# happykygo/GNN-eCommerce

Hardware: AMD Instinct MI355X
Metric: edges propagated/sec per LGConv layer (higher is better)
Workload: dtype f32; 1 GPU; configs[1]: 1639358 users x 54571 items, 20314816 directed edges, 3 LGConv layers, emb_dim 64, get_embedding (K hops + fused layer sum); parallelism=single, seed=0

## Files before the change

### gnn-ecommerce_amd/_native.py

```python
from __future__ import annotations

import ctypes
import os
from ctypes import CFUNCTYPE, POINTER, Structure, c_char_p, c_float, c_int, c_int32, c_int64, c_size_t, c_uint64, c_void_p
from typing import Optional

import torch

LIB_NAME = "liblgconv_hip.so"
LIB_PATH = os.environ.get("LGCN_LIB_PATH") or os.path.join(os.path.dirname(os.path.abspath(__file__)), "csrc", LIB_NAME)
ABI_VERSION = 14

ST_INDEX_OOB = 1
ST_SAMPLER_EXHAUSTED = 2

class SweepCfg(Structure):
    _fields_ = [("n_bands", c_int32), ("waves_per_band_round", c_int32), ("row_cap", c_int32), ("piece_cap", c_int32),
                ("lookahead", c_int32), ("groups", c_int32), ("round_order", c_int32), ("light_len", c_int32)]


class SweepDims(Structure):
    _fields_ = [("n_bands", c_int32), ("rounds", c_int32), ("row_cap", c_int32), ("piece_cap", c_int32),
                ("n_rows", c_int32), ("groups", c_int32),
                ("n_waves", c_int64), ("n_slabs", c_int64), ("n_slots", c_int64), ("n_entries", c_int64),
# ... 57 lines not shown
                                    c_int64, c_void_p]),
    "lgc_bipartite_split": (c_int, [c_void_p, c_int64, c_void_p, c_void_p]),
    "lgc_row_plan_workspace_bytes": (c_size_t, [c_int64]),
    "lgc_row_plan_count": (c_int, [c_void_p, c_int32, c_int32, c_int32, c_int32, c_void_p, c_size_t, c_void_p, c_void_p]),
    "lgc_row_plan_fill": (c_int, [c_void_p, c_int32, c_int32, c_int32, c_int32, c_void_p, c_void_p, c_void_p, c_void_p]),
    "lgc_tile_classes_workspace_bytes": (c_size_t, [c_int64, c_int64]),
    "lgc_tile_classes": (c_int, [c_void_p, c_void_p, c_int32, c_int32, c_int32, c_int32, c_int64, c_void_p, c_size_t, c_void_p,
                                 c_void_p, c_void_p]),
    "lgc_tile_pack": (c_int, [c_void_p, c_void_p, c_int64, c_int32, c_void_p, c_void_p, c_void_p]),
    "lgc_build_tiles": (c_int, [c_void_p, c_void_p, c_void_p, c_int64, c_int32, c_void_p, c_void_p]),
    "lgc_spmm_tiles": (c_int, [c_void_p, c_void_p, c_void_p, c_int32, c_int32, c_int32, c_int64, c_void_p, c_int64,
                               c_void_p, c_int64, c_void_p, c_int64, c_float, c_float, c_int32, c_void_p]),
    "lgc_sweep_plan_create": (c_void_p, [c_void_p, c_void_p, c_int32, c_int32, c_int32, c_int32, POINTER(SweepCfg),
                                         POINTER(c_int)]),
    "lgc_sweep_plan_dims": (c_int, [c_void_p, POINTER(SweepDims)]),
    "lgc_sweep_plan_export": (c_int, [c_void_p, c_void_p, c_void_p, c_void_p, c_void_p, c_void_p]),
    "lgc_sweep_plan_upload": (c_int, [c_void_p, c_void_p, c_void_p, c_void_p, c_void_p, c_void_p]),
    "lgc_sweep_plan_export_multi": (c_int, [c_void_p, c_void_p]),
    "lgc_sweep_plan_free": (None, [c_void_p]),
    "lgc_sweep_dplan_workspace_bytes": (c_size_t, [c_int64, c_int64, c_int64, POINTER(SweepCfg)]),
    "lgc_sweep_dplan_create": (c_void_p, [c_void_p, c_void_p, c_int32, c_int32, c_int64, c_int64, c_int32, c_int32,
                                          POINTER(SweepCfg), c_void_p, c_size_t, c_void_p, POINTER(c_int)]),
    "lgc_sweep_dplan_dims": (c_int, [c_void_p, POINTER(SweepDims)]),
    "lgc_sweep_dplan_fill": (c_int, [c_void_p, c_void_p, c_void_p, c_void_p, c_void_p, c_void_p]),
    "lgc_sweep_dplan_export_multi": (c_int, [c_void_p, c_void_p]),
    "lgc_sweep_dplan_free": (None, [c_void_p]),
    "lgc_sweep_ok": (c_int, [c_int32, c_int64, c_int64]),
    "lgc_spmm_sweep": (c_int, [c_void_p, c_void_p, c_void_p, c_void_p, c_int64, c_int32, c_int32, c_void_p, c_int32, c_void_p,
                               c_int32, c_void_p, c_int64, c_void_p, c_int64, c_void_p, c_int64, c_void_p, c_int64, c_float, c_float,
                               c_int32, c_void_p]),
    "lgc_apply_route": (c_int, [POINTER(OperatorC), c_int64, c_int64, c_int64, c_int64, c_int32]),
    "lgc_apply": (c_int, [POINTER(OperatorC), c_int64, c_void_p, c_int64, c_void_p, c_int64, c_void_p, c_int64, c_float, c_float,
                          c_int32, c_void_p]),
    "lgc_hop_exchange": (c_int, [POINTER(OperatorC), POINTER(OperatorC), c_int64, c_void_p, c_int64, c_void_p, c_int64, c_void_p,
                                 c_int64, c_float, c_float, c_int32, c_int32, c_int32, c_int32, EXCHANGE_FN, c_void_p, c_void_p]),
    "lgc_segment_sum": (c_int, [c_void_p, c_void_p, c_void_p, c_void_p, c_int64, c_float, c_void_p, c_int64, c_int64, c_int32,
                                c_int32, c_void_p]),
    "lgc_pair_dot_rows": (c_int, [c_void_p, c_int64, c_int32, c_int64, c_void_p, c_void_p, c_int64, c_void_p, c_void_p, c_void_p,
                                  c_void_p, c_void_p, c_void_p]),
    "lgc_reg_rows": (c_int, [c_void_p, c_int64, c_int32, c_int64, c_void_p, c_int64, c_void_p, c_int64, c_void_p, c_int64, c_float,
                             c_void_p, c_void_p, c_void_p, c_void_p]),
    "lgc_bpr_loss": (c_int, [c_void_p, c_void_p, c_int64, c_int64, c_void_p, c_void_p, c_void_p]),
    "lgc_pair_seed_vals": (c_int, [c_void_p, c_void_p, c_void_p, c_void_p, c_void_p, c_int64, c_int32, c_void_p, c_void_p]),
    "lgc_seed_prepare": (c_int, [c_void_p, c_int64, c_int64, c_int64, c_void_p, c_void_p, c_void_p, c_void_p, c_void_p, c_void_p,
                                 c_void_p, c_void_p, c_void_p]),
    "lgc_seed_flags": (c_int, [c_void_p, c_int64, c_int64, c_void_p, c_int32, c_void_p]),
    "lgc_seed_pull": (c_int, [c_void_p, c_void_p, c_int32, c_int32, c_int32, c_void_p, c_int32, c_void_p, c_int32, c_void_p,
                              c_void_p, c_void_p, c_void_p, c_void_p, c_int64, c_int64, c_void_p, c_int64, c_int32, c_void_p]),
    "lgc_seed_mark": (c_int, [c_void_p, c_void_p, c_int32, c_int32, c_void_p, c_int64, c_void_p, c_int64, c_int32, c_void_p]),
    "lgc_adam_step": (c_int, [c_void_p, c_void_p, c_void_p, c_void_p, c_int64, c_float, c_float, c_float, c_float, c_float,
                              c_float, c_void_p]),
    "lgc_adam_step_hp": (c_int, [c_void_p, c_void_p, c_void_p, c_void_p, c_int64, c_void_p, c_void_p]),
    "lgc_lincomb": (c_int, [c_void_p, c_int64, c_void_p, c_void_p, c_void_p, c_int32, c_int64, c_int32, c_void_p]),
    "lgc_mask_topk": (c_int, [c_void_p, c_int64, c_void_p, c_int64, c_void_p, c_void_p, c_void_p, c_int64, c_int32, c_int32,
                              c_void_p, c_void_p, c_void_p]),
    "lgc_fold_in": (c_int, [c_void_p, c_void_p, c_void_p, c_int64, c_void_p, c_void_p, c_int64, c_int64, c_void_p, c_void_p,
                            c_int64, c_int64, c_float, c_int32, c_int32, c_void_p, c_int64, c_void_p, c_void_p]),
    "lgc_score_rows": (c_int, [c_void_p, c_int64, c_int64, c_void_p, c_int64, c_void_p, c_int64, c_int32, c_int32, c_void_p,
                               c_int64, c_void_p, c_void_p]),
    "lgc_topk_hits": (c_int, [c_void_p, c_int64, c_int32, c_void_p, c_void_p, c_void_p, c_int64, c_int64, c_void_p, c_void_p,
                              c_void_p, c_void_p]),
    "lgc_metric_sums": (c_int, [c_void_p, c_void_p, c_int64, c_void_p, c_void_p, c_void_p]),
    "lgc_rank_metrics": (c_int, [c_void_p, c_int64, c_int32, c_void_p, c_void_p, c_void_p, c_void_p, c_int64, c_int64,
                                 POINTER(c_int32), c_int32, c_void_p, c_void_p, c_void_p, c_void_p, c_void_p]),
    "lgc_column_sums": (c_int, [c_void_p, c_int64, c_int64, c_int32, c_void_p, c_void_p]),
    "lgc_topk_coverage": (c_int, [c_void_p, c_int64, c_int32, c_int64, POINTER(c_int32), c_int32, c_int64, c_void_p, c_void_p,
# ... 130 lines not shown
```

### gnn-ecommerce_amd/csrc/lgconv_hip.hip

```cpp
#include <hipcub/hipcub.hpp>

#include <cstdlib>
#include <cstdio>
#include <cstring>
#include <chrono>
#include <new>
#include <thread>
#include <type_traits>
#include <utility>
#include <vector>

#include "lgconv_common.h"

namespace {

__global__ void k_build_keys(const int64_t *__restrict__ edge_index, int64_t n_edges, int64_t n_nodes,
                             int by_source, int32_t *__restrict__ keys, int32_t *__restrict__ ids,
                             int32_t *__restrict__ status) {
    int64_t e = (int64_t)blockIdx.x * blockDim.x + threadIdx.x;
    if (e >= n_edges) return;
    int64_t src = edge_index[e], dst = edge_index[n_edges + e];
    bool ok = src >= 0 && src < n_nodes && dst >= 0 && dst < n_nodes;
    if (!ok) atomicOr(status, LGC_ST_INDEX_OOB);
    keys[e] = ok ? (int32_t)(by_source ? src : dst) : 0;
// ... 1192 lines not shown
        __syncthreads();
        if (wv == 0 && active && g == 0) {
            for (int o = 1; o < kBlock / kWave; ++o) {
#pragma unroll
                for (int i = 0; i < VEC; ++i) acc.v[i] = __fadd_rn(acc.v[i], wave_sum[o * 256 + l * VEC + i]);
            }
            Acc<VEC> rv;
            rv.zero();
            if (p.r != nullptr) rv = load_row<VEC>(p.r + (int64_t)mr.row * p.r_stride + c0);
            finish_row<VEC, SpmmArgs>(p, mr.row, c0, acc, rv);
        }
        return;
    }
    const int64_t m = (((int64_t)blockIdx.x - n_wide) * (kBlock / kWave) + wv) * groups + g;
    if (g >= groups || m >= n_multi) return;
    const lgc_multi_row mr = multi[m];
    Acc<VEC> acc, rv;
    acc.zero();
    rv.zero();
    if (p.r != nullptr) rv = load_row<VEC>(p.r + (int64_t)mr.row * p.r_stride + c0);
    for (int32_t s = mr.slot_begin; s < mr.slot_end; s += 8) {
        Acc<VEC> t[8];
#pragma unroll
        for (int j = 0; j < 8; ++j) {
            t[j].zero();
            if (s + j < mr.slot_end) t[j] = load_row<VEC>(pb + (int64_t)(s + j) * p.dim);
        }
#pragma unroll
        for (int j = 0; j < 8; ++j)
#pragma unroll
            for (int i = 0; i < VEC; ++i) acc.v[i] = __fadd_rn(acc.v[i], t[j].v[i]);
    }
    finish_row<VEC, SpmmArgs>(p, mr.row, c0, acc, rv);
}

__global__ void k_seed_mark(const int32_t *__restrict__ rowptr, const lgc_entry *__restrict__ entries, int32_t row_begin,
                            int32_t row_end, const int64_t *__restrict__ seed_rows, int64_t n_seed, uint8_t *__restrict__ mark,
                            int64_t mark_len, uint8_t value) {
    const int lane = threadIdx.x & (kWave - 1);
    const int64_t t = (int64_t)blockIdx.x * (blockDim.x / kWave) + threadIdx.x / kWave;
    if (t >= n_seed) return;
    const int64_t row = seed_rows[t];
    if (row < row_begin || row >= row_end) return;
    if (t > 0 && seed_rows[t - 1] == row) return;
    for (int32_t k = rowptr[row] + lane; k < rowptr[row + 1]; k += kWave) {
        const int32_t c = entries[k].col;
        if (c >= 0 && c < mark_len) mark[c] = value;
    }
}

__global__ void k_split_init(long long *__restrict__ out) {
    out[0] = -1;
    out[1] = 0x7FFFFFFFFFFFFFFFll;
}

__global__ __launch_bounds__(kBlock) void k_bipartite_split(const int64_t *__restrict__ edge_index, int64_t n_edges,
                                                           long long *__restrict__ out) {
    long long lo = -1, hi = 0x7FFFFFFFFFFFFFFFll;
    for (int64_t e = (int64_t)blockIdx.x * blockDim.x + threadIdx.x; e < n_edges; e += (int64_t)gridDim.x * blockDim.x) {
        const long long a = edge_index[e], b = edge_index[n_edges + e];
        lo = max(lo, min(a, b));
        hi = min(hi, max(a, b));
    }
#pragma unroll
    for (int off = kWave / 2; off > 0; off >>= 1) {
        lo = max(lo, (long long)__shfl_xor(lo, off));
// ... 1388 lines not shown
    };
    int rc = up(wave_slab_ptr, plan->wave_slab_ptr.data(), plan->wave_slab_ptr.size() * 4);
    if (rc == 0) rc = up(wave_npieces, plan->wave_npieces.data(), plan->wave_npieces.size() * 4);
    if (rc == 0) rc = up(piece_slot, plan->piece_slot.data(), plan->piece_slot.size() * 4);
    if (rc != 0) return rc;
    const lgc_sweep_cfg &cfg = plan->cfg;
    const int64_t n_waves = plan->dims.n_waves;
    if (n_waves > 0 && plan->dims.n_entries > 0) {
        const uint32_t pad_x = 0x00FFFFFFu | ((uint32_t)cfg.row_cap << 24);
        hipLaunchKernelGGL((k_dp_steps<true>), dim3(ceil_div(n_waves, kBlock / kWave)), dim3(kBlock), 0, st, plan->keys, plan->idx,
                           plan->sorted, plan->d_item_ptr, (int32_t)n_waves, plan->dims.groups, cfg.lookahead,
                           cfg.waves_per_band_round, cfg.n_bands, cfg.round_order == 2 ? 1 : 0, pad_x, (int32_t *)nullptr,
                           (int32_t *)nullptr, (const int32_t *)wave_slab_ptr, slabs);
    }
    rc = (int)hipGetLastError();
    if (rc != 0) return rc;
    return (int)hipStreamSynchronize(st);
}

void lgc_sweep_dplan_free(lgc_sweep_dplan *plan) { delete plan; }

static bool sweep_table_ok(int32_t dim, int64_t table_rows, int64_t x_stride) {
    if (table_rows <= 0 || table_rows >= 0xFFFFFF || x_stride < dim) return false;
    const int64_t bytes = table_bytes(table_rows, x_stride, dim);
    const uint32_t pad = (uint32_t)(0xFFFFFFull * (uint64_t)(x_stride * 4));
    return x_stride * 4 < (1 << 24) && bytes < (int64_t(1) << 32) && (int64_t)pad >= bytes;
}

int lgc_sweep_ok(int32_t dim, int64_t table_rows, int64_t x_stride) {
    const int groups = (dim >= 61 && dim <= 64) ? 4 : (dim >= 68 && dim <= kWideRow) ? 2 : (dim > kWideRow && dim <= 128) ? 4 : 0;
    return groups != 0 && sweep_table_ok(dim, table_rows, x_stride) ? groups : 0;
}

int lgc_spmm_sweep(const uint32_t *slabs, const int32_t *wave_slab_ptr, const int32_t *wave_npieces, const int32_t *piece_slot,
                   int64_t n_waves, int32_t row_cap, int32_t groups, const lgc_multi_row *multi, int32_t n_rows,
                   const lgc_multi_row *multi_wide, int32_t n_wide, float *partials,
                   int64_t table_rows, const float *x, int64_t x_stride, float *y, int64_t y_stride, const float *r,
                   int64_t r_stride, float a, float b, int32_t dim, void *stream_) {
    if (!slabs || !wave_slab_ptr || !wave_npieces || !piece_slot || !partials || !x || !y || n_waves < 0 ||
        n_waves % 4 != 0 || n_rows < 0 || n_wide < 0 || (n_rows > 0 && !multi) || (n_wide > 0 && !multi_wide) || row_cap < 1 ||
        row_cap > 254 || x == y)
        return LGC_E_INVAL;
    if (groups == 0) groups = 4;
    if (lgc_sweep_ok(dim, table_rows, x_stride) != groups) return LGC_E_DIM;
    if (const int rc = check_tables(x, x_stride, y, y_stride, r, r_stride, dim)) return rc;
    if (!aligned_to(slabs, 16) || !aligned_to(partials, 16)) return LGC_E_ALIGN;
    hipStream_t stream = as_stream(stream_);
    const size_t lds = (size_t)(kBlock / kWave) * (size_t)(row_cap + 1) * (groups == 2 ? kWideRow : 64) * sizeof(float);
    if (lds > 160 * 1024) return LGC_E_INVAL;
    if (n_waves > 0) {
        SweepArgs p{reinterpret_cast<const u4 *>(slabs), wave_slab_ptr, wave_npieces, piece_slot, x, partials, x_stride,
                    (uint32_t)table_bytes(table_rows, x_stride, dim), dim, row_cap, (int32_t)n_waves, 0, nullptr, dim, 0};
        const bool two_pass = groups == 4 && dim > 64;
        if (two_pass) {
            p.dim = 64;
            p.x_bytes = (uint32_t)table_bytes(table_rows, x_stride, 64);
        }
#ifdef LGC_SWEEP_TRACE
        if (const char *tr = getenv("LGCN_SWEEP_TRACE")) p.trace = reinterpret_cast<unsigned long long *>(strtoull(tr, nullptr, 0));
#endif
        static unsigned long long lds_ok_sweep = 0, lds_ok_wide = 0;
        int rc_attr = allow_big_lds(reinterpret_cast<const void *>(k_sweep<kSweepDepth>), 160 * 1024, &lds_ok_sweep);
        if (rc_attr == 0) rc_attr = allow_big_lds(reinterpret_cast<const void *>(k_sweep_wide<8>), 160 * 1024, &lds_ok_wide);
        if (rc_attr != 0) return rc_attr;
        const int64_t req = knobs().sweep_launch_waves;
        const int64_t per_launch = req > 0 ? std::max<int64_t>(4, (req / 4) * 4) : n_waves;
        for (int64_t w0 = 0; w0 < n_waves; w0 += per_launch) {
            p.wave_begin = (int32_t)w0;
            const unsigned blocks = (unsigned)(std::min<int64_t>(per_launch, n_waves - w0) / 4);
            if (groups == 2) hipLaunchKernelGGL(k_sweep_wide<8>, dim3(blocks), dim3(kBlock), lds, stream, p);
            else hipLaunchKernelGGL(k_sweep<kSweepDepth>, dim3(blocks), dim3(kBlock), lds, stream, p);
            if (two_pass) {
                SweepArgs q = p;
                q.x = x + 64;
                q.dim = dim - 64;
                q.x_bytes = (uint32_t)table_bytes(table_rows, x_stride, dim - 64);
                q.pcol = 64;
                hipLaunchKernelGGL(k_sweep<kSweepDepth>, dim3(blocks), dim3(kBlock), lds, stream, q);
            }
        }
    }
    DimCfg cfg;
    dim_cfg(dim, &cfg);
    SpmmArgs sp{nullptr, nullptr, x, y, r, x_stride, y_stride, r_stride, a, b, dim, cfg.lpr, 0, 0, 0, 0};
    sp.wt_store = wt_store_ok(table_rows, y_stride) ? 1 : 0;
    if (n_wide + n_rows > 0) {
        const int rows_per_block = (kBlock / kWave) * (kWave / cfg.lpr);
        hipLaunchKernelGGL((k_sweep_combine<4>), dim3(n_wide + ceil_div(n_rows, rows_per_block)), dim3(kBlock), 0, stream, sp,
                           multi_wide, n_wide, multi, n_rows, partials);
    }
    return (int)hipGetLastError();
}

int lgc_apply_route(const lgc_operator *op, int64_t table_rows, int64_t x_stride, int64_t y_stride, int64_t r_stride,
                    int32_t dim) {
    if (!op || op->n_tile_classes < 0 || op->n_tile_classes > 3) return LGC_E_INVAL;
    DimCfg cfg;
    if (!dim_cfg(dim, &cfg)) return LGC_E_DIM;
    if (table_rows < 0 || x_stride < dim || y_stride < dim || r_stride < 0 || (r_stride > 0 && r_stride < dim)) return LGC_E_INVAL;
    const int wt = wt_store_ok(table_rows, y_stride) ? LGC_ROUTE_WT_STORE : 0;
    if (op->sweep) {
        const int groups = op->sweep->groups ? op->sweep->groups : 4;
        if (lgc_sweep_ok(dim, table_rows, x_stride) == groups)
            return wt | (groups == 2 ? LGC_ROUTE_SWEEP_WIDE : dim > 64 ? LGC_ROUTE_SWEEP_TWO_PASS : LGC_ROUTE_SWEEP);
    }
    if (op->n_tile_classes == 0 || dim < 4) return wt | LGC_ROUTE_ROWS;
    bool fast = true;
    for (int c = 0; c < op->n_tile_classes; ++c)
        if (op->tiles[c].n_tiles != 0)
            fast = fast && tiles_fast_ok(op->tiles[c].meta != nullptr, dim, table_rows, x_stride, y_stride, r_stride);
    if (knobs().no_fused_apply) return wt | (fast ? LGC_ROUTE_SPLIT_DPP : LGC_ROUTE_SPLIT_GENERIC);
    return wt | (fast ? LGC_ROUTE_FUSED_DPP : LGC_ROUTE_FUSED_GENERIC);
}

int lgc_apply(const lgc_operator *op, int64_t table_rows, const float *x, int64_t x_stride, float *y, int64_t y_stride,
              const float *r, int64_t r_stride, float a, float b, int32_t dim, void *stream) {
    const int route = lgc_apply_route(op, table_rows, x_stride, y_stride, r ? r_stride : 0, dim);
    if (route < 0) return route;
    if (r && r_stride < dim) return LGC_E_INVAL;
    switch (route & ~LGC_ROUTE_WT_STORE) {
    case LGC_ROUTE_SWEEP:
    case LGC_ROUTE_SWEEP_WIDE:
    case LGC_ROUTE_SWEEP_TWO_PASS: {
        const lgc_sweep_arrays *sw = op->sweep;
// ... 35 lines not shown
        hipStream_t st = as_stream(stream);
        if (total > 0) {
            if (fast && dim > 64) hipLaunchKernelGGL((k_apply_fused<2>), dim3((unsigned)total), dim3(kBlock), 0, st, f);
            else if (fast) hipLaunchKernelGGL((k_apply_fused<1>), dim3((unsigned)total), dim3(kBlock), 0, st, f);
            else hipLaunchKernelGGL((k_apply_fused<0>), dim3((unsigned)total), dim3(kBlock), 0, st, f);
        }
        if (op->n_multi > 0)
            hipLaunchKernelGGL((k_spmm_combine<4>), dim3(ceil_div(op->n_multi, kBlock / kWave)), dim3(kBlock), 0, st, f.sp, op->multi,
                               op->n_multi, op->partials);
        return (int)hipGetLastError();
    }
    default:
        break;
    }
    const bool tiled = (route & ~LGC_ROUTE_WT_STORE) != LGC_ROUTE_ROWS;
    if (!tiled || op->n_chunks > 0) {
        const int rc = lgc_spmm(op->rowptr, op->entries, op->row_begin, tiled ? op->row_begin : op->row_end, op->short_max,
                                op->chunks, op->n_chunks, op->multi, op->n_multi, op->partials, table_rows, x, x_stride, y,
                                y_stride, r, r_stride, a, b, dim, stream);
        if (rc != 0) return rc;
    }
    if (tiled) {
        for (int c = 0; c < op->n_tile_classes; ++c) {
            const lgc_tile_class &tc = op->tiles[c];
            const int rc = lgc_spmm_tiles(tc.order, tc.meta, tc.slab, tc.n_tiles, tc.width,
                                          op->tiles_per_wave > 0 ? op->tiles_per_wave : 1, table_rows, x, x_stride, y,
                                          y_stride, r, r_stride, a, b, dim, stream);
            if (rc != 0) return rc;
        }
    }
    return 0;
}

int lgc_hop_exchange(const lgc_operator *item_op, const lgc_operator *user_op, int64_t table_rows, const float *x,
                     int64_t x_stride, float *y, int64_t y_stride, const float *r, int64_t r_stride, float a, float b,
                     int32_t dim, int32_t exchange_row_begin, int32_t exchange_rows, int32_t item_epilogue,
                     lgc_exchange_fn exchange, void *user, void *stream) {
    if (!item_op || !user_op || !exchange || exchange_row_begin < 0 || exchange_rows < 0 ||
        (int64_t)exchange_row_begin + exchange_rows > table_rows)
        return LGC_E_INVAL;
    int rc = lgc_apply(item_op, table_rows, x, x_stride, y, y_stride, item_epilogue ? r : nullptr, item_epilogue ? r_stride : 0, a,
                       item_epilogue ? b : 0.0f, dim, stream);
    if (rc != 0) return rc;
    rc = exchange(y + (int64_t)exchange_row_begin * y_stride, exchange_rows, y_stride, dim, stream, user);
    if (rc != 0) return rc;
    return lgc_apply(user_op, table_rows, x, x_stride, y, y_stride, r, r_stride, a, b, dim, stream);
}

int lgc_seed_mark(const int32_t *rowptr, const lgc_entry *entries, int32_t row_begin, int32_t row_end, const int64_t *seed_rows,
                  int64_t n_seed, uint8_t *mark, int64_t mark_len, int32_t value, void *stream_) {
    if (n_seed < 0 || row_begin < 0 || row_end < row_begin || mark_len < 0 || value < 0 || value > 255) return LGC_E_INVAL;
    if (n_seed == 0) return 0;
    if (!rowptr || !entries || !seed_rows || !mark) return LGC_E_INVAL;
    hipLaunchKernelGGL(k_seed_mark, dim3(ceil_div(n_seed, (int64_t)(kBlock / kWave))), dim3(kBlock), 0, as_stream(stream_), rowptr, entries,
                       row_begin, row_end, seed_rows, n_seed, mark, mark_len, (uint8_t)value);
    return (int)hipGetLastError();
}

int lgc_seed_pull(const int32_t *rowptr, const lgc_entry *entries, int32_t row_begin, int32_t row_end, int32_t short_max,
                  const lgc_chunk *chunks, int32_t n_chunks, const lgc_multi_row *multi, int32_t n_multi, float *partials,
                  const uint8_t *col_flag, const int32_t *col_slot, const uint8_t *row_mark, const float *seed_vals,
                  int64_t seed_stride, int64_t table_rows, float *y, int64_t y_stride, int32_t dim, void *stream_) {
    DimCfg cfg;
    if (!dim_cfg(dim, &cfg)) return LGC_E_DIM;
    if (!rowptr || !col_flag || !col_slot || row_begin < 0 || row_end < row_begin || n_chunks < 0 || n_multi < 0 ||
        short_max < 0 || table_rows < row_end)
// ... 50 lines not shown
```

### gnn-ecommerce_amd/graph.py

```python
from __future__ import annotations

import os
from collections import OrderedDict
from dataclasses import dataclass, field
from typing import Callable, Dict, List, Optional, Tuple

import torch
from torch import Tensor

from . import _native

SHORT_MAX = int(os.environ.get("LGCN_SHORT_MAX", "32"))
CHUNK_LEN = int(os.environ.get("LGCN_CHUNK_LEN", "256"))
USER_CHUNK_LEN = int(os.environ.get("LGCN_USER_CHUNK_LEN", "4096"))
TILE_WIDTHS = (8, 16, 32)
USE_TILES = os.environ.get("LGCN_TILES", "1") == "1"
TILES_PER_WAVE = int(os.environ.get("LGCN_TILES_PER_WAVE", "1"))
TILE_ORDER = os.environ.get("LGCN_TILE_ORDER", "cold")
USE_SWEEP = os.environ.get("LGCN_SWEEP", "auto")
SWEEP_MIN_ENTRIES = int(os.environ.get("LGCN_SWEEP_MIN_ENTRIES", "1000000"))
SWEEP_ADAPTIVE_BANDS = os.environ.get("LGCN_SWEEP_ADAPTIVE_BANDS", "1") == "1"
SWEEP_PIECE_ENTRIES = int(os.environ.get("LGCN_SWEEP_PIECE_ENTRIES", "20"))
SWEEP_CFG = dict(n_bands=int(os.environ.get("LGCN_SWEEP_BANDS", "8")), waves_per_band_round=int(os.environ.get("LGCN_SWEEP_WAVES", "256")),
                 row_cap=int(os.environ.get("LGCN_SWEEP_ROW_CAP", "78")),
# ... 488 lines not shown
                                      _native.ptr(sw.piece_slot), _native.ptr(sw.multi) if sw.multi.size(0) else None,
                                      _native.ptr(sw.multi_wide) if sw.multi_wide.size(0) else None,
                                      _native.ptr(sw.partials(dim)), sw.dims["n_waves"], sw.dims["row_cap"], sw.multi.size(0),
                                      sw.multi_wide.size(0), sw.dims["groups"])
            c.sweep = ctypes.pointer(sc)
            keep.append(sc)
        self._c_structs[key] = keep
        return c

    def _apply_args(self, x: Tensor, out: Tensor, r: Optional[Tensor]):
        _check_table(x, "x")
        _check_table(out, "out")
        dim = x.size(1)
        if out.size(1) != dim or (r is not None and r.size(1) != dim):
            raise ValueError("x, out and r must have the same width")
        if out.data_ptr() == x.data_ptr():
            raise ValueError("out must not alias x")
        if r is not None:
            _check_table(r, "r")
        lib = _native.load()
        if not lib.lgc_dim_ok(dim):
            raise _native.NativeLibraryError(f"embedding width {dim} is not supported by the HIP kernels")
        table_rows = min(x.size(0), out.size(0))
        sweep = sweep_choice(lib, dim, table_rows, x.stride(0)) if self.sweep_cols is not None else 0
        return lib, self.c_struct(dim, sweep), dim, table_rows

    def route(self, x: Tensor, out: Tensor, r: Optional[Tensor] = None) -> str:
        import ctypes
        lib, c, dim, table_rows = self._apply_args(x, out, r)
        code = lib.lgc_apply_route(ctypes.byref(c), table_rows, x.stride(0), out.stride(0), 0 if r is None else r.stride(0), dim)
        _native.check(min(code, 0), "lgc_apply_route")
        return _native.route_name(code)

    def apply(self, x: Tensor, out: Tensor, a: float = 1.0, r: Optional[Tensor] = None, b: float = 0.0) -> Tensor:
        import ctypes
        lib, c, dim, table_rows = self._apply_args(x, out, r)
        with torch.cuda.device(x.device):
            code = lib.lgc_apply(ctypes.byref(c), table_rows, _native.ptr(x), x.stride(0), _native.ptr(out), out.stride(0),
                                 _native.ptr(r), 0 if r is None else r.stride(0), float(a), float(b), dim,
                                 _native.stream_of(x.device))
        _native.check(code, "lgc_apply")
        return out


_rows_scratch: Dict[tuple, Tuple[Tensor, Tensor]] = {}
LISTED_ROWS_MAX_SHARE = float(os.environ.get("LGCN_LISTED_ROWS_MAX_SHARE", "0.4"))


def row_stats(rowptr: Tensor, row_begin: int, row_end: int) -> Tuple[float, float, int]:
    deg = (rowptr[row_begin + 1:row_end + 1] - rowptr[row_begin:row_end]).double()
    s1, s2 = torch.stack((deg.sum(), (deg * deg).sum())).tolist()
    return s1, s2, max(row_end - row_begin, 1)


def listed_rows_pay(stats: Tuple[float, float, int], n_ids: int) -> bool:
    s1, s2, rows = stats
    if s1 <= 0:
        return True
    return n_ids / 4.0 * (s2 / s1 + s1 / rows) <= LISTED_ROWS_MAX_SHARE * s1


ROWS_SPLIT_ROOM = 16384


def _rows_split_scratch(device: torch.device, n_ids: int, dim: int) -> Tuple[Tensor, Tensor]:
    import threading
    key = (device, torch.cuda.current_stream(device).cuda_stream, threading.get_ident(), dim)
    got = _rows_scratch.get(key)
    if got is None or got[0].numel() < n_ids + 2:
# ... 17 lines not shown
    if out.size(1) != dim or (r is not None and r.size(1) != dim):
        raise ValueError("x, out and r must have the same width")
    if compact and not split:
        raise ValueError("compact output needs split=True")
    rows = rows.contiguous()
    lib = _native.load()
    p = op.plan
    n_ids = rows.numel()
    with torch.cuda.device(x.device):
        if split:
            if n_ids == 0:
                return out
            if out.size(0) < (n_ids if compact else p.row_end):
                raise ValueError("out has too few rows")
            work, partials = _rows_split_scratch(x.device, n_ids, dim)
            code = lib.lgc_spmm_rows_split(_native.ptr(op.rowptr), _native.ptr(op.entries), p.row_begin, p.row_end, _native.ptr(rows),
                                           n_ids, x.size(0), _native.ptr(x), x.stride(0), _native.ptr(out), out.stride(0),
                                           out.size(0), _native.ptr(r), 0 if r is None else r.stride(0), float(a), float(b), dim,
                                           int(compact), _native.ptr(work), _native.ptr(partials), partials.size(0),
                                           _native.stream_of(x.device))
            _native.check(code, "lgc_spmm_rows_split")
            return out
        code = lib.lgc_spmm_rows(_native.ptr(op.rowptr), _native.ptr(op.entries), p.row_begin, p.row_end, _native.ptr(rows),
                                 n_ids, min(x.size(0), out.size(0)), _native.ptr(x), x.stride(0), _native.ptr(out),
                                 out.stride(0), _native.ptr(r), 0 if r is None else r.stride(0), float(a), float(b), dim,
                                 _native.stream_of(x.device))
    _native.check(code, "lgc_spmm_rows")
    return out


ELIMINATE_MAX_DEG = os.environ.get("LGCN_ELIMINATE_MAX_DEG", "auto")
ELIMINATE_AUTO_MAX_DEG = int(os.environ.get("LGCN_ELIMINATE_AUTO_MAX_DEG", "3"))
ELIMINATE_MAX_GRAM_SHARE = float(os.environ.get("LGCN_ELIMINATE_MAX_GRAM_SHARE", "1.0"))
GRAM_CHUNK_LEN = int(os.environ.get("LGCN_GRAM_CHUNK_LEN", "256"))


@dataclass
class ReducedCSR:
    max_deg: int
    n_h: int
    n_items: int
    user_map: Tensor
    rowptr: Tensor
    entries: Tensor
    user_nnz: int
    n_pairs: int
    gram_rowptr: Tensor
    gram_entries: Tensor

    @property
    def nnz(self) -> int:
        return self.entries.size(0)

    @property
    def gram_nnz(self) -> int:
        return self.gram_entries.size(0)


def build_reduced_csr(rowptr: Tensor, entries: Tensor, split: int, num_nodes: int, max_deg: int) -> Optional[ReducedCSR]:
    lib = _native.load()
    _native.require_device(rowptr, "rowptr")
    dev = rowptr.device
    n_edges = entries.size(0)
    n_items = num_nodes - split
    u8 = dict(dtype=torch.uint8, device=dev)
    i32 = dict(dtype=torch.int32, device=dev)
# ... 187 lines not shown

    def _find_bipartite_split(self) -> Optional[int]:
        if self.num_edges == 0:
            return None
        out = torch.empty(2, dtype=torch.int64, device=self.device)
        lib = _native.load()
        with torch.cuda.device(self.device):
            code = lib.lgc_bipartite_split(_native.ptr(self._edge_index), self.num_edges, _native.ptr(out),
                                           _native.stream_of(self.device))
        _native.check(code, "lgc_bipartite_split")
        lo, hi = out.tolist()
        return lo + 1 if lo < hi else None

    def halves(self, transpose: bool = False) -> Tuple[Operator, Operator]:
        if self.split is None:
            raise ValueError("graph is not bipartite")
        got = self._halves.get(transpose)
        if got is None:
            op = self.transpose_op if transpose else self.forward_op
            got = tuple(Operator.build(op.n_rows, op.rowptr, op.entries, lo, hi, self.short_max, chunk, sweep_cols=cols)
                        for (lo, hi), cols, chunk in (((0, self.split), (self.split, self.num_nodes),
                                                       max(self.chunk_len, USER_CHUNK_LEN)),
                                                      ((self.split, self.num_nodes), (0, self.split), self.chunk_len)))
            self._halves[transpose] = got
        return got

    eliminate_max_deg: Optional[int] = None

    def reduced(self, transpose: bool = False) -> Optional[ReducedGraph]:
        if transpose or self.split is None:
            return None
        forced = self.eliminate_max_deg
        auto = forced is None and ELIMINATE_MAX_DEG == "auto"
        max_deg = int(forced) if forced is not None else (ELIMINATE_AUTO_MAX_DEG if auto else int(ELIMINATE_MAX_DEG))
        if max_deg <= 0:
            return None
        key = ("reduced", max_deg, auto)
        if key in self._halves:
            return self._halves[key]
        got = None
        if not auto or self.halves(False)[1].sweep_cols is not None:
            got = self._build_reduced(max_deg)
            if got is not None and auto:
                removed = self.forward_op.nnz - got.csr.nnz
                if got.csr.gram_nnz > ELIMINATE_MAX_GRAM_SHARE * removed:
                    got = None
        self._halves[key] = got
        return got

    def _build_reduced(self, max_deg: int) -> Optional[ReducedGraph]:
        op = self.forward_op
        csr = build_reduced_csr(op.rowptr, op.entries, self.split, self.num_nodes, max_deg)
        if csr is None:
            return None
        n_h, n_rows = csr.n_h, csr.n_h + csr.n_items
        user_chunk = max(self.chunk_len, USER_CHUNK_LEN)
        user_op_h = item_op_h = gram_op = None
        if n_h > 0:
            user_op_h = Operator.build(n_rows, csr.rowptr, csr.entries, 0, n_h, self.short_max, user_chunk,
                                       sweep_cols=(n_h, n_rows))
        if csr.nnz - csr.user_nnz > 0:
            item_op_h = Operator.build(n_rows, csr.rowptr, csr.entries, n_h, n_rows, self.short_max, self.chunk_len,
                                       sweep_cols=(0, n_h))
        if csr.gram_nnz > 0:
            gram_op = Operator.build(n_rows, csr.gram_rowptr, csr.gram_entries, n_h, n_rows, self.short_max, GRAM_CHUNK_LEN)

        def concat() -> Optional[ConcatGraph]:
            n_gaps = int(SWEEP_CFG["n_bands"])
            n_phys = int(_native.load().lgc_reduce_concat_rows(n_h, csr.n_items, n_gaps))
            if csr.gram_nnz == 0 or n_phys < 0 or n_phys > self.split:
                return None
            cc = build_concat_csr(csr, n_gaps)
            rows = n_phys + csr.n_items
            return ConcatGraph(cc, self.split - n_phys,
                               Operator.build(rows, cc.rowptr, cc.entries, 0, n_phys, self.short_max, user_chunk,
                                              sweep_cols=(n_phys, rows)),
                               Operator.build(rows, cc.rowptr, cc.entries, n_phys, rows, self.short_max, self.chunk_len,
                                              sweep_cols=(0, n_phys)))
# ... 161 lines not shown
```

### gnn-ecommerce_amd/propagate.py

```python
from __future__ import annotations

import os
from typing import List, Optional, Sequence

import torch
from torch import Tensor
from torch.autograd.function import once_differentiable

from . import _native
from .graph import Operator, PropGraph, apply_rows


HOP_EVENT_LOG: Optional[list] = None


def _timed_apply(op: Operator, x: Tensor, out: Tensor, **kw) -> None:
    if HOP_EVENT_LOG is None:
        op.apply(x, out, **kw)
        return
    start, end = torch.cuda.Event(enable_timing=True), torch.cuda.Event(enable_timing=True)
    start.record()
    op.apply(x, out, **kw)
    end.record()
    HOP_EVENT_LOG.append((start, end))
# ... 51 lines not shown
    tables = [x0]
    red = reduced if k >= 2 else None
    rows_items_only = final_rows is not None and SCORED_ITEM_ROWS_ONLY and item_op.listed_rows_pay(final_rows.numel()) \
        if red is not None else False

    cc = red.concat_for(x0.size(1), n, x0.size(1) if (not PAD_INTERNAL or x0.size(1) % 32 == 0)
                        else (x0.size(1) + 31) // 32 * 32) if red is not None else None

    def user_step(layer: int, x: Tensor, out_t: Tensor) -> None:
        if red is None or (rows_items_only and layer == k - 1):
            user_op.apply(x, out_t)
        elif cc is not None:
            cc.user_op.apply(x[cc.offset:], out_t[cc.offset:])
        elif red.user_op_h is not None:
            red.user_op_h.apply(x[red.offset:], out_t[red.offset:])

    def item_step(layer: int, out_t: Tensor, a: float = 1.0, r: Optional[Tensor] = None) -> None:
        if cc is not None:
            o = cc.offset
            cc.item_op.apply(tables[layer - 1][o:], out_t[o:], a=a, r=None if r is None else r[o:], b=0.0 if r is None else 1.0)
            return
        o = red.offset
        y = out_t[o:]
        have = r is not None
        if red.gram_op is not None:
            red.gram_op.apply(tables[layer - 2][o:], y, a=a, r=r[o:] if have else None, b=1.0 if have else 0.0)
        elif have:
            _native.lincomb(out_t[split:], [(1.0, r[split:])])
        else:
            out_t[split:].zero_()
        if red.item_op_h is not None:
            red.item_op_h.apply(tables[layer - 1][o:], y, a=a, r=y, b=1.0)
    uniform = UNIFORM_ALPHA_SHORTCUT and all(a == alphas[0] for a in alphas) and (UNIFORM_ALPHA_SHORTCUT == "force" or x0.size(1) % 32 == 0)
    for layer in range(1, k + 1):
        with _HopSpan():
            nxt = scratch_table(x0)
            if layer < k:
                if red is None or layer == 1:
                    item_op.apply(tables[-1], nxt)
                else:
                    item_step(layer, nxt)
                user_step(layer, tables[-1], nxt)
                tables.append(nxt)
            else:
                out = torch.empty_like(x0)
                rows_only = final_rows is not None
                if rows_only and SCORED_ITEM_ROWS_ONLY and item_op.listed_rows_pay(final_rows.numel()):
                    mix = nxt
                    _native.lincomb(mix[split:], [(alphas[l], tables[l - 1][split:]) for l in range(1, k + 1)])
                    if all(a == alphas[0] for a in alphas):
                        rest = mix
                    else:
                        rest = scratch_table(x0)
                        _native.lincomb(rest[split:], [(alphas[l], tables[l][split:]) for l in range(0, k)])
                    apply_rows(item_op, final_rows, tables[-1], out, a=alphas[k], r=rest, b=1.0, split=True)
                elif uniform:
                    mix = nxt
                    _native.lincomb(mix[split:], [(alphas[l], tables[l - 1][split:]) for l in range(1, k + 1)])
                    if red is None:
                        item_op.apply(tables[-1], out, a=alphas[k], r=mix, b=1.0)
                    else:
                        item_step(k, out, a=alphas[k], r=mix)
                else:
                    if red is None:
                        item_op.apply(tables[-1], nxt)
                    else:
                        item_step(k, nxt)
                    tables.append(nxt)
                    mix = scratch_table(x0)
                    _native.lincomb(mix[split:], [(alphas[l], tables[l - 1][split:]) for l in range(1, k + 1)])
                    _native.lincomb(out[split:], [(alphas[l], tables[l][split:]) for l in range(0, k + 1)])
                if not rows_only:
                    user_op.apply(mix, out, a=1.0, r=x0, b=alphas[0])
                else:
                    apply_rows(user_op, final_rows, mix, out, a=1.0, r=x0, b=alphas[0])
    return out


def _layer_sum(graph: PropGraph, x: Tensor, alphas: tuple, transpose: bool, final_rows: Optional[Tensor] = None) -> Tensor:
    if USE_BIPARTITE and graph.split is not None and len(alphas) - 1 <= _native.MAX_TERMS - 1:
        user_op, item_op = graph.halves(transpose)
        return bipartite_sum(user_op, item_op, graph.split, x, alphas, final_rows if SCORED_ROWS_ONLY else None,
                             reduced=graph.reduced(transpose) if len(alphas) > 2 else None)
    return horner_hops(graph.transpose_op if transpose else graph.forward_op, x, alphas)


UNIFORM_ALPHA_SHORTCUT = {"0": False, "force": "force"}.get(os.environ.get("LGCN_UNIFORM_ALPHA_SHORTCUT", "1"), True)
SCORED_ROWS_ONLY = os.environ.get("LGCN_SCORED_ROWS_ONLY", "1") == "1"
SCORED_ITEM_ROWS_ONLY = os.environ.get("LGCN_SCORED_ITEM_ROWS_ONLY", "1") == "1"


class _PropagateSum(torch.autograd.Function):
    @staticmethod
    def forward(ctx, x0: Tensor, graph: PropGraph, alphas: tuple) -> Tensor:
        ctx.graph, ctx.alphas = graph, alphas
        return _layer_sum(graph, x0.detach(), alphas, transpose=False)

    @staticmethod
    @once_differentiable
    def backward(ctx, grad_out: Tensor):
        return _layer_sum(ctx.graph, grad_out.contiguous(), ctx.alphas, transpose=True), None, None


class _Hop(torch.autograd.Function):

    @staticmethod
    def forward(ctx, x: Tensor, graph: PropGraph) -> Tensor:
        ctx.graph = graph
        x = x.detach().contiguous()
        return graph.forward_op.apply(x, torch.empty_like(x))

    @staticmethod
    @once_differentiable
    def backward(ctx, grad_out: Tensor):
        g = grad_out.contiguous()
        return ctx.graph.transpose_op.apply(g, torch.empty_like(g)), None


def propagate_sum(x0: Tensor, graph: PropGraph, alphas: Sequence[float]) -> Tensor:
    _native.require_device(x0, "embedding table")
# ... 1017 lines not shown
```

### include/lgconv_hip.h

```cpp
#ifndef LGCONV_HIP_H
#define LGCONV_HIP_H

#include <stddef.h>
#include <stdint.h>

#ifdef __cplusplus
extern "C" {
#endif

#define LGC_ABI_VERSION 14

#define LGC_E_INVAL      (-1)
#define LGC_E_DIM        (-2)
#define LGC_E_WORKSPACE  (-3)
#define LGC_E_RANGE      (-4)
#define LGC_E_ALIGN      (-5)

#define LGC_ST_INDEX_OOB 1

typedef struct lgc_entry {
    int32_t col;
    float   val;
} lgc_entry;

// ... 130 lines not shown

typedef struct lgc_tile_class {
    const int32_t   *order;
    const int32_t   *meta;
    const lgc_entry *slab;
    int32_t n_tiles, width;
} lgc_tile_class;

typedef struct lgc_sweep_arrays {
    const uint32_t *slabs;
    const int32_t  *wave_slab_ptr, *wave_npieces, *piece_slot;
    const lgc_multi_row *multi, *multi_wide;
    float   *partials;
    int64_t  n_waves;
    int32_t  row_cap, n_rows, n_wide;
    int32_t  groups;
} lgc_sweep_arrays;

typedef struct lgc_operator {
    const int32_t   *rowptr;
    const lgc_entry *entries;
    const lgc_chunk *chunks;
    const lgc_multi_row *multi;
    float   *partials;
    const lgc_sweep_arrays *sweep;
    lgc_tile_class tiles[3];
    int32_t row_begin, row_end, short_max, n_chunks, n_multi, n_tile_classes, tiles_per_wave, reserved;
} lgc_operator;

int lgc_apply_route(const lgc_operator *op, int64_t table_rows, int64_t x_stride, int64_t y_stride, int64_t r_stride,
                    int32_t dim);
int lgc_apply(const lgc_operator *op, int64_t table_rows, const float *x, int64_t x_stride, float *y, int64_t y_stride,
              const float *r, int64_t r_stride, float a, float b, int32_t dim, void *stream);

typedef int (*lgc_exchange_fn)(float *block, int64_t rows, int64_t row_stride, int32_t dim, void *stream, void *user);

int lgc_hop_exchange(const lgc_operator *item_op, const lgc_operator *user_op, int64_t table_rows, const float *x,
                     int64_t x_stride, float *y, int64_t y_stride, const float *r, int64_t r_stride, float a, float b,
                     int32_t dim, int32_t exchange_row_begin, int32_t exchange_rows, int32_t item_epilogue,
                     lgc_exchange_fn exchange, void *user, void *stream);

int lgc_segment_sum(const int64_t *key_sorted, const int64_t *dest, const float *vals, const int32_t *vals_index, int64_t n,
                    float scale, float *y, int64_t y_stride, int64_t y_rows, int32_t dim, int32_t accumulate, void *stream);

#define LGC_SEED_MAX 8192
int lgc_pair_dot_rows(const float *emb, int64_t stride, int32_t dim, int64_t n_nodes, const int64_t *idx0, const int64_t *idx1,
                      int64_t n_pairs, float *scores, float *rows0, float *rows1, uint8_t *ok, int32_t *status, void *stream);
int lgc_bpr_loss(const float *scores, const uint8_t *mask, int64_t n_triples, int64_t size, float *loss, float *grad,
                 void *stream);
int lgc_reg_rows(const float *w, int64_t stride, int32_t dim, int64_t n_rows, const int64_t *ids0, int64_t m0, const int64_t *ids1,
                 int64_t m1, const int64_t *ids2, int64_t m2, float scale, float *value, int64_t *rows_out, int32_t *status,
                 void *stream);

int lgc_pair_seed_vals(const float *grad_scores, const uint8_t *mask, const float *grad_scale, const float *rows0,
                       const float *rows1, int64_t n_pairs, int32_t dim, float *vals, void *stream);
int lgc_seed_prepare(const int64_t *rows, int64_t m, int64_t split, int64_t n_nodes, int64_t *rows_sorted, int32_t *perm,
                     int64_t *dest_item, int64_t *dest_slot, int64_t *dest_user, uint8_t *col_flag, int32_t *col_slot,
                     uint64_t *scratch , void *stream);
int lgc_seed_flags(const int64_t *rows_sorted, int64_t m, int64_t split, uint8_t *col_flag, int32_t value, void *stream);

int lgc_seed_pull(const int32_t *rowptr, const lgc_entry *entries, int32_t row_begin, int32_t row_end, int32_t short_max,
                  const lgc_chunk *chunks, int32_t n_chunks, const lgc_multi_row *multi, int32_t n_multi, float *partials,
                  const uint8_t *col_flag, const int32_t *col_slot, const uint8_t *row_mark, const float *seed_vals,
                  int64_t seed_stride, int64_t table_rows, float *y, int64_t y_stride, int32_t dim, void *stream);

int lgc_seed_mark(const int32_t *rowptr, const lgc_entry *entries, int32_t row_begin, int32_t row_end, const int64_t *seed_rows,
// ... 152 lines not shown
```

Baseline: 40.76 billion edges/s.

## Fuse layer-sum mixing into item sweep epilogue with second residual row

Adds a sweep-combine kernel variant and an lgc_apply2 entry point whose epilogue computes a*acc + b*r + b2*r2. With uniform alphas and K of 2 or 3, this lets the penultimate item hop produce the weighted layer mix directly, so the separate lincomb over item rows and one scratch table are skipped. It also raises the auto thresholds for degree elimination when reduced concat mode is on, which allows more low-degree nodes to be eliminated. The propagation control flow becomes more intricate, and the tables reused as the mix must keep the correct semantics.

```diff
diff --git a/gnn-ecommerce_amd/_native.py b/gnn-ecommerce_amd/_native.py
--- a/gnn-ecommerce_amd/_native.py
+++ b/gnn-ecommerce_amd/_native.py
@@ -113,6 +113,8 @@
     "lgc_apply_route": (c_int, [POINTER(OperatorC), c_int64, c_int64, c_int64, c_int64, c_int32]),
     "lgc_apply": (c_int, [POINTER(OperatorC), c_int64, c_void_p, c_int64, c_void_p, c_int64, c_void_p, c_int64, c_float, c_float,
                           c_int32, c_void_p]),
+    "lgc_apply2": (c_int, [POINTER(OperatorC), c_int64, c_void_p, c_int64, c_void_p, c_int64, c_void_p, c_int64, c_void_p, c_int64,
+                           c_float, c_float, c_float, c_int32, c_void_p]),
     "lgc_hop_exchange": (c_int, [POINTER(OperatorC), POINTER(OperatorC), c_int64, c_void_p, c_int64, c_void_p, c_int64, c_void_p,
                                  c_int64, c_float, c_float, c_int32, c_int32, c_int32, c_int32, EXCHANGE_FN, c_void_p, c_void_p]),
     "lgc_segment_sum": (c_int, [c_void_p, c_void_p, c_void_p, c_void_p, c_int64, c_float, c_void_p, c_int64, c_int64, c_int32,
diff --git a/gnn-ecommerce_amd/csrc/lgconv_hip.hip b/gnn-ecommerce_amd/csrc/lgconv_hip.hip
--- a/gnn-ecommerce_amd/csrc/lgconv_hip.hip
+++ b/gnn-ecommerce_amd/csrc/lgconv_hip.hip
@@ -1248,6 +1248,105 @@
             for (int i = 0; i < VEC; ++i) acc.v[i] = __fadd_rn(acc.v[i], t[j].v[i]);
     }
     finish_row<VEC, SpmmArgs>(p, mr.row, c0, acc, rv);
+}
+
+struct EpilogueRow2 {
+    const float *r2;
+    int64_t r2_stride;
+    float b2;
+};
+
+template <int VEC>
+__device__ __forceinline__ void finish_row2(const SpmmArgs &p, const EpilogueRow2 &q, int64_t row, int c0, Acc<VEC> acc,
+                                            const Acc<VEC> &rv, const Acc<VEC> &r2v) {
+    if (p.a != 1.0f) {
+#pragma unroll
+        for (int i = 0; i < VEC; ++i) acc.v[i] = __fmul_rn(p.a, acc.v[i]);
+    }
+#pragma unroll
+    for (int i = 0; i < VEC; ++i)
+        acc.v[i] = __fadd_rn(__fadd_rn(__fmul_rn(q.b2, r2v.v[i]), __fmul_rn(p.b, rv.v[i])), acc.v[i]);
+    store_out<VEC, SpmmArgs>(p, row, c0, acc);
+}
+
+template <int VEC>
+__global__ __launch_bounds__(kBlock) void k_sweep_combine2(SpmmArgs p, const lgc_multi_row *__restrict__ wide, int32_t n_wide,
+                                                          const lgc_multi_row *__restrict__ multi, int32_t n_multi,
+                                                          const float *__restrict__ partials, EpilogueRow2 q) {
+    __shared__ float wave_sum[(kBlock / kWave) * 256];
+    const int lane = threadIdx.x & (kWave - 1);
+    const int wv = threadIdx.x / kWave;
+    const int groups = kWave / p.lpr;
+    const int g = lane / p.lpr;
+    const int l = lane - g * p.lpr;
+    const int c0 = lane_column<VEC>(l, p.dim);
+    const float *pb = partials + c0;
+    if ((int32_t)blockIdx.x < n_wide) {
+        const lgc_multi_row mr = wide[blockIdx.x];
+        const bool active = g < groups;
+        const int units = (kBlock / kWave) * groups;
+        Acc<VEC> acc;
+        acc.zero();
+        if (active) {
+            int32_t s = mr.slot_begin + wv * groups + g;
+            for (; s + 3 * units < mr.slot_end; s += 4 * units) {
+                Acc<VEC> t0 = load_row<VEC>(pb + (int64_t)s * p.dim);
+                Acc<VEC> t1 = load_row<VEC>(pb + (int64_t)(s + units) * p.dim);
+                Acc<VEC> t2 = load_row<VEC>(pb + (int64_t)(s + 2 * units) * p.dim);
+                Acc<VEC> t3 = load_row<VEC>(pb + (int64_t)(s + 3 * units) * p.dim);
+#pragma unroll
+                for (int i = 0; i < VEC; ++i)
+                    acc.v[i] = __fadd_rn(__fadd_rn(__fadd_rn(__fadd_rn(acc.v[i], t0.v[i]), t1.v[i]), t2.v[i]), t3.v[i]);
+            }
+            for (; s < mr.slot_end; s += units) {
+                Acc<VEC> t0 = load_row<VEC>(pb + (int64_t)s * p.dim);
+#pragma unroll
+                for (int i = 0; i < VEC; ++i) acc.v[i] = __fadd_rn(acc.v[i], t0.v[i]);
+            }
+        }
+        for (int j = 1; j < groups; ++j) {
+#pragma unroll
+            for (int i = 0; i < VEC; ++i) {
+                float other = __shfl_down(acc.v[i], j * p.lpr);
+                if (g == 0) acc.v[i] = __fadd_rn(acc.v[i], other);
+            }
+        }
+        if (active && g == 0) {
+#pragma unroll
+            for (int i = 0; i < VEC; ++i) wave_sum[wv * 256 + l * VEC + i] = acc.v[i];
+        }
+        __syncthreads();
+        if (wv == 0 && active && g == 0) {
+            for (int o = 1; o < kBlock / kWave; ++o) {
+#pragma unroll
+                for (int i = 0; i < VEC; ++i) acc.v[i] = __fadd_rn(acc.v[i], wave_sum[o * 256 + l * VEC + i]);
+            }
+            const Acc<VEC> r2v = load_row<VEC>(q.r2 + (int64_t)mr.row * q.r2_stride + c0);
+            const Acc<VEC> rv = load_row<VEC>(p.r + (int64_t)mr.row * p.r_stride + c0);
+            finish_row2<VEC>(p, q, mr.row, c0, acc, rv, r2v);
+        }
+        return;
+    }
+    const int64_t m = (((int64_t)blockIdx.x - n_wide) * (kBlock / kWave) + wv) * groups + g;
+    if (g >= groups || m >= n_multi) return;
+    const lgc_multi_row mr = multi[m];
+    Acc<VEC> acc;
+    acc.zero();
+    const Acc<VEC> r2v = load_row<VEC>(q.r2 + (int64_t)mr.row * q.r2_stride + c0);
+    const Acc<VEC> rv = load_row<VEC>(p.r + (int64_t)mr.row * p.r_stride + c0);
+    for (int32_t s = mr.slot_begin; s < mr.slot_end; s += 8) {
+        Acc<VEC> t[8];
+#pragma unroll
+        for (int j = 0; j < 8; ++j) {
+            t[j].zero();
+            if (s + j < mr.slot_end) t[j] = load_row<VEC>(pb + (int64_t)(s + j) * p.dim);
+        }
+#pragma unroll
+        for (int j = 0; j < 8; ++j)
+#pragma unroll
+            for (int i = 0; i < VEC; ++i) acc.v[i] = __fadd_rn(acc.v[i], t[j].v[i]);
+    }
+    finish_row2<VEC>(p, q, mr.row, c0, acc, rv, r2v);
 }
 
 __global__ void k_seed_mark(const int32_t *__restrict__ rowptr, const lgc_entry *__restrict__ entries, int32_t row_begin,
@@ -2702,11 +2801,14 @@
     return groups != 0 && sweep_table_ok(dim, table_rows, x_stride) ? groups : 0;
 }
 
-int lgc_spmm_sweep(const uint32_t *slabs, const int32_t *wave_slab_ptr, const int32_t *wave_npieces, const int32_t *piece_slot,
-                   int64_t n_waves, int32_t row_cap, int32_t groups, const lgc_multi_row *multi, int32_t n_rows,
-                   const lgc_multi_row *multi_wide, int32_t n_wide, float *partials,
-                   int64_t table_rows, const float *x, int64_t x_stride, float *y, int64_t y_stride, const float *r,
-                   int64_t r_stride, float a, float b, int32_t dim, void *stream_) {
+static int spmm_sweep(const uint32_t *slabs, const int32_t *wave_slab_ptr, const int32_t *wave_npieces, const int32_t *piece_slot,
+                      int64_t n_waves, int32_t row_cap, int32_t groups, const lgc_multi_row *multi, int32_t n_rows,
+                      const lgc_multi_row *multi_wide, int32_t n_wide, float *partials,
+                      int64_t table_rows, const float *x, int64_t x_stride, float *y, int64_t y_stride, const float *r,
+                      int64_t r_stride, const float *r2, int64_t r2_stride, float a, float b, float b2, int32_t dim,
+                      void *stream_) {
+    if (r2 && (!r || r2_stride < dim)) return LGC_E_INVAL;
+    if (r2 && !aligned_to(r2, 4)) return LGC_E_ALIGN;
     if (!slabs || !wave_slab_ptr || !wave_npieces || !piece_slot || !partials || !x || !y || n_waves < 0 ||
         n_waves % 4 != 0 || n_rows < 0 || n_wide < 0 || (n_rows > 0 && !multi) || (n_wide > 0 && !multi_wide) || row_cap < 1 ||
         row_cap > 254 || x == y)
@@ -2756,10 +2858,23 @@
     sp.wt_store = wt_store_ok(table_rows, y_stride) ? 1 : 0;
     if (n_wide + n_rows > 0) {
         const int rows_per_block = (kBlock / kWave) * (kWave / cfg.lpr);
-        hipLaunchKernelGGL((k_sweep_combine<4>), dim3(n_wide + ceil_div(n_rows, rows_per_block)), dim3(kBlock), 0, stream, sp,
-                           multi_wide, n_wide, multi, n_rows, partials);
+        const dim3 grid(n_wide + ceil_div(n_rows, rows_per_block));
+        if (r2)
+            hipLaunchKernelGGL((k_sweep_combine2<4>), grid, dim3(kBlock), 0, stream, sp, multi_wide, n_wide, multi, n_rows, partials,
+                               EpilogueRow2{r2, r2_stride, b2});
+        else
+            hipLaunchKernelGGL((k_sweep_combine<4>), grid, dim3(kBlock), 0, stream, sp, multi_wide, n_wide, multi, n_rows, partials);
     }
     return (int)hipGetLastError();
+}
+
+int lgc_spmm_sweep(const uint32_t *slabs, const int32_t *wave_slab_ptr, const int32_t *wave_npieces, const int32_t *piece_slot,
+                   int64_t n_waves, int32_t row_cap, int32_t groups, const lgc_multi_row *multi, int32_t n_rows,
+                   const lgc_multi_row *multi_wide, int32_t n_wide, float *partials,
+                   int64_t table_rows, const float *x, int64_t x_stride, float *y, int64_t y_stride, const float *r,
+                   int64_t r_stride, float a, float b, int32_t dim, void *stream_) {
+    return spmm_sweep(slabs, wave_slab_ptr, wave_npieces, piece_slot, n_waves, row_cap, groups, multi, n_rows, multi_wide, n_wide,
+                      partials, table_rows, x, x_stride, y, y_stride, r, r_stride, nullptr, 0, a, b, 0.0f, dim, stream_);
 }
 
 int lgc_apply_route(const lgc_operator *op, int64_t table_rows, int64_t x_stride, int64_t y_stride, int64_t r_stride,
@@ -2861,6 +2976,26 @@
     return 0;
 }
 
+int lgc_apply2(const lgc_operator *op, int64_t table_rows, const float *x, int64_t x_stride, float *y, int64_t y_stride,
+               const float *r, int64_t r_stride, const float *r2, int64_t r2_stride, float a, float b, float b2, int32_t dim,
+               void *stream) {
+    const int route = lgc_apply_route(op, table_rows, x_stride, y_stride, r ? r_stride : 0, dim);
+    if (route < 0) return route;
+    if (!r || r_stride < dim || !r2 || r2_stride < dim) return LGC_E_INVAL;
+    switch (route & ~LGC_ROUTE_WT_STORE) {
+    case LGC_ROUTE_SWEEP:
+    case LGC_ROUTE_SWEEP_WIDE:
+    case LGC_ROUTE_SWEEP_TWO_PASS: {
+        const lgc_sweep_arrays *sw = op->sweep;
+        return spmm_sweep(sw->slabs, sw->wave_slab_ptr, sw->wave_npieces, sw->piece_slot, sw->n_waves, sw->row_cap, sw->groups,
+                          sw->multi, sw->n_rows, sw->multi_wide, sw->n_wide, sw->partials, table_rows, x, x_stride, y, y_stride, r,
+                          r_stride, r2, r2_stride, a, b, b2, dim, stream);
+    }
+    default:
+        return LGC_E_DIM;
+    }
+}
+
 int lgc_hop_exchange(const lgc_operator *item_op, const lgc_operator *user_op, int64_t table_rows, const float *x,
                      int64_t x_stride, float *y, int64_t y_stride, const float *r, int64_t r_stride, float a, float b,
                      int32_t dim, int32_t exchange_row_begin, int32_t exchange_rows, int32_t item_epilogue,
diff --git a/gnn-ecommerce_amd/graph.py b/gnn-ecommerce_amd/graph.py
--- a/gnn-ecommerce_amd/graph.py
+++ b/gnn-ecommerce_amd/graph.py
@@ -544,9 +544,25 @@
         _native.check(min(code, 0), "lgc_apply_route")
         return _native.route_name(code)
 
-    def apply(self, x: Tensor, out: Tensor, a: float = 1.0, r: Optional[Tensor] = None, b: float = 0.0) -> Tensor:
+    def takes_second_row(self, x: Tensor, out: Tensor, r: Tensor) -> bool:
+        return self.route(x, out, r).split("+")[0] in ("sweep", "sweep_wide", "sweep_two_pass")
+
+    def apply(self, x: Tensor, out: Tensor, a: float = 1.0, r: Optional[Tensor] = None, b: float = 0.0,
+              r2: Optional[Tensor] = None, b2: float = 0.0) -> Tensor:
         import ctypes
         lib, c, dim, table_rows = self._apply_args(x, out, r)
+        if r2 is not None:
+            if r is None:
+                raise ValueError("r2 needs r")
+            _check_table(r2, "r2")
+            if r2.size(1) != dim:
+                raise ValueError("x, out, r and r2 must have the same width")
+            with torch.cuda.device(x.device):
+                code = lib.lgc_apply2(ctypes.byref(c), table_rows, _native.ptr(x), x.stride(0), _native.ptr(out), out.stride(0),
+                                      _native.ptr(r), r.stride(0), _native.ptr(r2), r2.stride(0), float(a), float(b), float(b2),
+                                      dim, _native.stream_of(x.device))
+            _native.check(code, "lgc_apply2")
+            return out
         with torch.cuda.device(x.device):
             code = lib.lgc_apply(ctypes.byref(c), table_rows, _native.ptr(x), x.stride(0), _native.ptr(out), out.stride(0),
                                  _native.ptr(r), 0 if r is None else r.stride(0), float(a), float(b), dim,
@@ -630,6 +646,8 @@
 ELIMINATE_MAX_DEG = os.environ.get("LGCN_ELIMINATE_MAX_DEG", "auto")
 ELIMINATE_AUTO_MAX_DEG = int(os.environ.get("LGCN_ELIMINATE_AUTO_MAX_DEG", "3"))
 ELIMINATE_MAX_GRAM_SHARE = float(os.environ.get("LGCN_ELIMINATE_MAX_GRAM_SHARE", "1.0"))
+ELIMINATE_AUTO_MAX_DEG_CONCAT = int(os.environ.get("LGCN_ELIMINATE_AUTO_MAX_DEG_CONCAT", "4"))
+ELIMINATE_MAX_GRAM_SHARE_CONCAT = float(os.environ.get("LGCN_ELIMINATE_MAX_GRAM_SHARE_CONCAT", "1.25"))
 GRAM_CHUNK_LEN = int(os.environ.get("LGCN_GRAM_CHUNK_LEN", "256"))
 
 
@@ -883,7 +901,10 @@
             return None
         forced = self.eliminate_max_deg
         auto = forced is None and ELIMINATE_MAX_DEG == "auto"
-        max_deg = int(forced) if forced is not None else (ELIMINATE_AUTO_MAX_DEG if auto else int(ELIMINATE_MAX_DEG))
+        concat = REDUCED_CONCAT != "0"
+        auto_deg, auto_share = ((ELIMINATE_AUTO_MAX_DEG_CONCAT, ELIMINATE_MAX_GRAM_SHARE_CONCAT) if concat else
+                                (ELIMINATE_AUTO_MAX_DEG, ELIMINATE_MAX_GRAM_SHARE))
+        max_deg = int(forced) if forced is not None else (auto_deg if auto else int(ELIMINATE_MAX_DEG))
         if max_deg <= 0:
             return None
         key = ("reduced", max_deg, auto)
@@ -894,7 +915,7 @@
             got = self._build_reduced(max_deg)
             if got is not None and auto:
                 removed = self.forward_op.nnz - got.csr.nnz
-                if got.csr.gram_nnz > ELIMINATE_MAX_GRAM_SHARE * removed:
+                if got.csr.gram_nnz > auto_share * removed:
                     got = None
         self._halves[key] = got
         return got
diff --git a/gnn-ecommerce_amd/propagate.py b/gnn-ecommerce_amd/propagate.py
--- a/gnn-ecommerce_amd/propagate.py
+++ b/gnn-ecommerce_amd/propagate.py
@@ -107,11 +107,34 @@
         if red.item_op_h is not None:
             red.item_op_h.apply(tables[layer - 1][o:], y, a=a, r=y, b=1.0)
     uniform = UNIFORM_ALPHA_SHORTCUT and all(a == alphas[0] for a in alphas) and (UNIFORM_ALPHA_SHORTCUT == "force" or x0.size(1) % 32 == 0)
+
+    def mix_in_item_step(out_t: Tensor) -> bool:
+        if not (MIX_IN_ITEM_STEP and uniform and final_rows is None and k in (2, 3)):
+            return False
+        if red is None or k == 2:
+            op, o = item_op, 0
+        elif cc is not None:
+            op, o = cc.item_op, cc.offset
+        else:
+            return False
+        x = tables[k - 2][o:]
+        if not op.takes_second_row(x, out_t[o:], x):
+            return False
+        assert op.sweep_cols is not None and o + op.sweep_cols[1] <= split
+        if k == 2:
+            op.apply(x, out_t[o:], a=alphas[2], r=x, b=alphas[1])
+        else:
+            op.apply(x, out_t[o:], a=alphas[3], r=x, b=alphas[2], r2=tables[0][o:], b2=alphas[1])
+        return True
+
+    mixed = False
     for layer in range(1, k + 1):
         with _HopSpan():
-            nxt = scratch_table(x0)
+            nxt = None if mixed else scratch_table(x0)
             if layer < k:
-                if red is None or layer == 1:
+                if layer == k - 1 and mix_in_item_step(nxt):
+                    mixed = True
+                elif red is None or layer == 1:
                     item_op.apply(tables[-1], nxt)
                 else:
                     item_step(layer, nxt)
@@ -130,8 +153,11 @@
                         _native.lincomb(rest[split:], [(alphas[l], tables[l][split:]) for l in range(0, k)])
                     apply_rows(item_op, final_rows, tables[-1], out, a=alphas[k], r=rest, b=1.0, split=True)
                 elif uniform:
-                    mix = nxt
-                    _native.lincomb(mix[split:], [(alphas[l], tables[l - 1][split:]) for l in range(1, k + 1)])
+                    if mixed:
+                        mix = tables[-1]
+                    else:
+                        mix = nxt
+                        _native.lincomb(mix[split:], [(alphas[l], tables[l - 1][split:]) for l in range(1, k + 1)])
                     if red is None:
                         item_op.apply(tables[-1], out, a=alphas[k], r=mix, b=1.0)
                     else:
@@ -160,7 +186,8 @@
     return horner_hops(graph.transpose_op if transpose else graph.forward_op, x, alphas)
 
 
-UNIFORM_ALPHA_SHORTCUT = {"0": False, "force": "force"}.get(os.environ.get("LGCN_UNIFORM_ALPHA_SHORTCUT", "1"), True)
+MIX_IN_ITEM_STEP = os.environ.get("LGCN_MIX_IN_ITEM_STEP", "1") == "1"
+UNIFORM_ALPHA_SHORTCUT ={"0": False, "force": "force"}.get(os.environ.get("LGCN_UNIFORM_ALPHA_SHORTCUT", "1"), True)
 SCORED_ROWS_ONLY = os.environ.get("LGCN_SCORED_ROWS_ONLY", "1") == "1"
 SCORED_ITEM_ROWS_ONLY = os.environ.get("LGCN_SCORED_ITEM_ROWS_ONLY", "1") == "1"
 
diff --git a/include/lgconv_hip.h b/include/lgconv_hip.h
--- a/include/lgconv_hip.h
+++ b/include/lgconv_hip.h
@@ -186,6 +186,10 @@
                     int32_t dim);
 int lgc_apply(const lgc_operator *op, int64_t table_rows, const float *x, int64_t x_stride, float *y, int64_t y_stride,
               const float *r, int64_t r_stride, float a, float b, int32_t dim, void *stream);
+
+int lgc_apply2(const lgc_operator *op, int64_t table_rows, const float *x, int64_t x_stride, float *y, int64_t y_stride,
+               const float *r, int64_t r_stride, const float *r2, int64_t r2_stride, float a, float b, float b2, int32_t dim,
+               void *stream);
 
 typedef int (*lgc_exchange_fn)(float *block, int64_t rows, int64_t row_stride, int32_t dim, void *stream, void *user);
 
```

Result: faster. 41.80 billion edges/s (median of 6 runs) (+2.5%).
